# gyoge0/sub_volume_renderer

Measured on AMD Instinct MI355X. Metric: Mray-steps/sec (+ frames/sec) of the LMIP sub-volume march at 1920x1080, 3-LOD 1024^3 volume, higher is better.
Workload: dtype f32

## Files before the change

### sub_volume_renderer_amd/csrc/march_kernel.hip

```cpp
#include <stdlib.h>

#include <algorithm>
#include <type_traits>

#include "svr_internal.h"
#include "twin_address.h"
#include "slab_box.h"

namespace {

struct f3 { float x, y, z; };
struct f4 { float x, y, z, w; };

__device__ __forceinline__ f4 mat_vec(const float* m, float x, float y, float z, float w) {
    f4 r;
    r.x = ((m[0] * x + m[4] * y) + m[8]  * z) + m[12] * w;
    r.y = ((m[1] * x + m[5] * y) + m[9]  * z) + m[13] * w;
    r.z = ((m[2] * x + m[6] * y) + m[10] * z) + m[14] * w;
    r.w = ((m[3] * x + m[7] * y) + m[11] * z) + m[15] * w;
    return r;
}

__device__ __forceinline__ float dot3(f3 a, f3 b) { return (a.x * b.x + a.y * b.y) + a.z * b.z; }

// ... 467 lines not shown
                     SVR_STEP1X("quad_perm:[2,3,0,1] row_mask:0xf bank_mask:0xf")
                     SVR_STEP1X("row_half_mirror row_mask:0xf bank_mask:0xf")
                     SVR_STEP1X("row_mirror row_mask:0xf bank_mask:0xf")
                     SVR_STEP1X("row_bcast:15 row_mask:0xa bank_mask:0xf")
                     SVR_STEP1X("row_bcast:31 row_mask:0xc bank_mask:0xf")
                     "s_nop 0" : "+v"(v));
    else
        asm volatile(SVR_STEP1("quad_perm:[1,0,3,2] row_mask:0xf bank_mask:0xf")
                     SVR_STEP1("quad_perm:[2,3,0,1] row_mask:0xf bank_mask:0xf")
                     SVR_STEP1("row_half_mirror row_mask:0xf bank_mask:0xf")
                     SVR_STEP1("row_mirror row_mask:0xf bank_mask:0xf")
                     SVR_STEP1("row_bcast:15 row_mask:0xa bank_mask:0xf")
                     SVR_STEP1("row_bcast:31 row_mask:0xc bank_mask:0xf")
                     "s_nop 0" : "+v"(v));
#undef SVR_STEP1
#undef SVR_STEP1X
    return __builtin_amdgcn_readlane(v, 63);
}

struct LodK {
    uint32_t ring[3];
    float    scale[3];
    int32_t  addw[3];
    uint32_t rx4, base_bytes;
    float    ss[3];
    int32_t  slab;
    const void* rbase;
    uint32_t rbytes;
    uint32_t nparts, zsplit, part_bytes, rbytes_last;
    uint32_t twin;
};
__device__ __forceinline__ LodK load_lod(kparams_t p, int l) {
    LodK k;
#pragma unroll
    for (int a = 0; a < 3; ++a) {
        k.ring[a] = p->lod[l].ring[a]; k.scale[a] = p->lod[l].scale[a]; k.addw[a] = p->lod[l].addw[a]; k.ss[a] = p->lod[l].ss[a];
    }
    k.rx4 = p->lod[l].rx4; k.base_bytes = p->lod[l].base_bytes; k.slab = p->lod[l].slab;
    k.rbase = p->lod[l].rbase; k.rbytes = p->lod[l].rbytes;
    k.nparts = p->lod[l].nparts; k.zsplit = p->lod[l].zsplit; k.part_bytes = p->lod[l].part_bytes; k.rbytes_last = p->lod[l].rbytes_last;
    k.twin = p->lod[l].twin;
    return k;
}

struct LodEvents {
    int a, b;
    int cx, cy, cz;
};


template <int NL, int U, bool COUNT, int ESH, bool BIG, bool WAVG = false, bool SCALED = false>
__global__ __launch_bounds__(256) __attribute__((amdgpu_waves_per_eu(SCALED && !COUNT ? 5 : 1))) void march_span(const MarchParams P) {
    static_assert(!(SCALED && WAVG), "the weighted-average reducer reads the unscaled step");
    extern __shared__ __attribute__((aligned(16))) uint8_t lds_all[];
    const int nblocks = P.tiles_x * P.tiles_y;
    const int tb = P.tile_order ? (int)P.tile_order[blockIdx.x] : xcd_remap((int)blockIdx.x, nblocks);
    const int tile_x = tb % P.tiles_x, tile_y = tb / P.tiles_x;
    const int wave = __builtin_amdgcn_readfirstlane((int)(threadIdx.x >> 6)), lane = threadIdx.x & 63;
    const int lw = P.tile_log2w, wl = P.block_waves_log2;
    const int c0 = ((tile_x << wl) + (wave & wl)) << lw, r0 = ((tile_y << wl) + (wave >> 1)) << (6 - lw);
    int lc = lane & ((1 << lw) - 1), lr = lane >> lw;
    {
        const float pcx = (float)(P.frame.x0 + c0) + 0.5f * (float)(1 << lw);
        const float pcy = (float)(P.frame.y0 + (r0 / P.frame.band_h) * P.frame.band_pitch + (r0 % P.frame.band_h)) +
                          0.5f * (float)(64 >> lw);
        const float ncx = 2.0f * pcx / (float)P.frame.frame_w - 1.0f;
        const float ncy = 1.0f - 2.0f * pcy / (float)P.frame.frame_h;
        const float dx = (P.xdir[0] - ncx * P.xdir[3]) * (float)P.frame.frame_w;
        const float dy = (P.xdir[1] - ncy * P.xdir[3]) * (float)P.frame.frame_h;
        if (P.orient && fabsf(dy) > fabsf(dx)) { lr = lane & ((64 >> lw) - 1); lc = lane >> (6 - lw); }
    }
    const int c = c0 + lc;
    const int r = r0 + lr;
    const bool inside = c < P.frame.out_w && r < P.frame.out_h;
    const size_t o = (size_t)r * (size_t)P.frame.out_w + (size_t)c;
    const int x = P.frame.x0 + c;
    const int y = P.frame.y0 + (r / P.frame.band_h) * P.frame.band_pitch + (r % P.frame.band_h);

    unsigned long long t_acc[16] = { 0, 0, 0, 0, 0, 0, 0, 0, 0, 0, 0, 0, 0, 0, 0, 0 };
    unsigned long long t_last = COUNT ? __builtin_amdgcn_s_memtime() : 0ull;
    auto lap = [&](int k) {
        if (COUNT) {
            const unsigned long long t = __builtin_amdgcn_s_memtime();
            t_acc[k] += t - t_last;
            t_last = t;
        }
    };

    Ray Rs;
    Rs.nsteps = 0; Rs.start = { 0.f, 0.f, 0.f }; Rs.step = { 0.f, 0.f, 0.f };
    const bool frag = inside && (x < P.frame.frame_w && y < P.frame.frame_h) && setup_ray(P, x, y, Rs);
    const int nsteps = frag ? Rs.nsteps : 0;
    float Rsx = frag ? Rs.start.x : 0.f, Rsy = frag ? Rs.start.y : 0.f, Rsz = frag ? Rs.start.z : 0.f;
    float Rtx = frag ? Rs.step.x : 0.f, Rty = frag ? Rs.step.y : 0.f, Rtz = frag ? Rs.step.z : 0.f;

    float d0[3], d1[3];
    {
        const float lastf = (float)(nsteps - 1);
        d0[0] = (Rsx + 0.0f * Rtx) * P.size[0];  d1[0] = (Rsx + lastf * Rtx) * P.size[0];
        d0[1] = (Rsy + 0.0f * Rty) * P.size[1];  d1[1] = (Rsy + lastf * Rty) * P.size[1];
        d0[2] = (Rsz + 0.0f * Rtz) * P.size[2];  d1[2] = (Rsz + lastf * Rtz) * P.size[2];
    }
    LodEvents ev[NL];
#pragma unroll
    for (int l = 0; l < NL; ++l) {
        const LodParams& L = P.lod[l];
        int a = 0, b = nsteps, cr[3] = { 0, 0, 0 };
        if (L.shape[0] == 0 || L.shape[1] == 0 || L.shape[2] == 0) {
            ev[l].a = 0; ev[l].b = 0; ev[l].cx = 0; ev[l].cy = 0; ev[l].cz = 0;
            continue;
        }
#pragma unroll
        for (int ax = 0; ax < 3; ++ax) {
            const float st = ax == 0 ? Rsx : (ax == 1 ? Rsy : Rsz);
            const float sp = ax == 0 ? Rtx : (ax == 1 ? Rty : Rtz);
            const bool inc = sp > 0.0f;
            const int v0 = (int)(d0[ax] * L.scale[ax]), v1 = (int)(d1[ax] * L.scale[ax]);
            auto cross = [&](int T) {
                const bool p0 = inc ? v0 >= T : v0 < T;
                const bool p1 = inc ? v1 >= T : v1 < T;
                int j = p0 ? 0 : nsteps;
                const bool need = !p0 && p1;
                if (__builtin_amdgcn_ballot_w64(need) != 0) {
                    const int js = first_cross(nsteps, st, sp, P.size[ax], L.scale[ax], T, need);
                    j = need ? js : j;
                }
                return j;
            };
            const int lo = L.off[ax], hi = L.off[ax] + (int)L.shape[ax];
            const int jlo = cross(lo);
            const int jhi = cross(hi);
            int en = inc ? jlo : jhi, ex = inc ? jhi : jlo;
            if (!(sp > 0.0f) && !(sp < 0.0f)) {
                en = 0; ex = (lo <= v0 && v0 < hi) ? nsteps : 0;
            }
            a = max(a, en); b = min(b, ex);
            if (L.wrap0[ax] + L.shape[ax] > L.ring[ax])
                cr[ax] = cross((int)L.ring[ax] - L.addw[ax]);
            else
                cr[ax] = inc ? nsteps : 0;
        }
        if (a >= b || L.shape[0] == 0) { a = 0; b = 0; }
        ev[l].a = a; ev[l].b = b; ev[l].cx = cr[0]; ev[l].cy = cr[1]; ev[l].cz = cr[2];
    }

    __amdgpu_buffer_rsrc_t rsrc_all = __builtin_amdgcn_make_buffer_rsrc(
        const_cast<void*>(P.density_all), 0, (int)P.density_all_bytes, 0x00020000);

#ifdef SVR_EXPERIMENTS
    const int dbg_nowait = P.dbg_nowait, brick_pow2 = P.brick_pow2;
#else
    constexpr int dbg_nowait = 0, brick_pow2 = 0;
#endif
    bool found = false, finished = (dbg_nowait & 2) != 0;
    float local_max = 0.f, samp = 0.f;
    int hit_i = 0, since = 0;
    uint32_t steps = 0;

    typedef typename Texel<ESH>::type texel_t;
    texel_t thr_raw;
    if constexpr (ESH != 2) thr_raw = P.lmip_threshold_raw; else thr_raw = P.lmip_threshold;
    const bool mip_like = (P.skip_flags & 2) != 0;
    float den = 0.f;
    auto lmip_batch = [&](const texel_t (&sv)[U], int nb, bool live, bool tail) {
        if constexpr (WAVG) {
            const float steplen = sqrtf((Rtx * Rtx + Rty * Rty) + Rtz * Rtz);
            const float k = fresh_params(P)->weight_falloff;
#pragma unroll
            for (int u = 0; u < U; ++u) {
                const bool act = live && !finished && (!tail || (nb + u) < nsteps);
                const float tw = 1.0f - k * ((float)(nb + u) * steplen);
                const bool go = act && tw > 0.0f;
                finished = finished || (act && !go);
                if (COUNT) steps += go ? 1u : 0u;
                const float val = texel_value(sv[u]);
                const float w = tw * tw;
                const float contribution = w * fabsf(val);
                const float num1 = samp + w * val, den1 = den + w;
                samp = go ? num1 : samp;
                den = go ? den1 : den;
                const bool take = go && contribution > local_max;
                local_max = take ? contribution : local_max;
                hit_i = take ? (nb + u) : hit_i;
            }
            return;
        }
        texel_t m;
        if constexpr (ESH != 2) m = 0u; else m = -1.0f;
        const texel_t neutral = m;
#pragma unroll
        for (int u = 0; u < U; ++u) m = texel_max(m, (tail && (nb + u) >= nsteps) ? neutral : texel_abs(sv[u]));
        bool need;
        if (mip_like) need = live && (found ? texel_value(m) > local_max : m >= thr_raw);
        else need = live && (found || m >= thr_raw);
        if (__builtin_amdgcn_ballot_w64(need) != 0) {
#pragma unroll
            for (int u = 0; u < U; ++u) {
                const bool act = live && !finished && (!tail || (nb + u) < nsteps);
                const float val = texel_value(sv[u]);
                const float inten = fabsf(val);
                if (COUNT) steps += act ? 1u : 0u;
                const bool was_found = found;
                const bool first_hit = act && !was_found && inten >= P.lmip_threshold;
                const bool tracking = act && was_found;
                since += tracking ? 1 : 0;
                const bool take = first_hit || (tracking && inten > local_max);
                local_max = take ? inten : local_max;
                samp = take ? val : samp;
                hit_i = take ? (nb + u) : hit_i;
                found = found || first_hit;
                const bool brk = tracking && (since >= P.lmip_max_samples || inten < local_max * P.lmip_fall_off);
                finished = finished || brk;
            }
        } else if (COUNT) {
            steps += live ? (uint32_t)(tail ? (min(nb + U, nsteps) - nb) : U) : 0u;
        }
    };

    int code = NL, E = 0;
    uint32_t Kc = 0xFFFFFFFFu;
    uint32_t Kb = 0u;
    int zth = 0;

    int brick_mode = 0;
    bool many_lines = false;
    if (P.brick) {
        const float pf = (float)min(max(nsteps - 1, 0), 256);
        const int qx = (int)((Rsx + pf * Rtx) * P.size[0]) >> (7 - ESH);
        const int qy = (int)((Rsy + pf * Rty) * P.size[1]);
        const int qz = (int)((Rsz + pf * Rtz) * P.size[2]);
        const int key = frag ? ((qz * 4099 + qy) * 64 + (qx & 63)) : -1 - lane;
        const int k0 = __builtin_amdgcn_update_dpp(key, key, 0x00, 0xF, 0xF, false);
        const int k1 = __builtin_amdgcn_update_dpp(key, key, 0x55, 0xF, 0xF, false);
        const int k2 = __builtin_amdgcn_update_dpp(key, key, 0xAA, 0xF, 0xF, false);
        const int q = lane & 3;
        const bool fresh = frag && (q == 0 || (key != k0 && (q == 1 || (key != k1 && (q == 2 || key != k2)))));
        const int lines = __builtin_popcountll(__builtin_amdgcn_ballot_w64(fresh));
        const int quads = __builtin_popcountll(__builtin_amdgcn_ballot_w64(frag && q == 0)) + 1;
        const bool use_brick = P.brick >= 2 || lines * 16 > P.brick_lines * quads;
        brick_mode = use_brick ? 1 + P.slab_long : 0;
        many_lines = use_brick;
    }
    const int wave_lds = wave * P.brick_bytes;

    int c_general = 0, c_direct = 0, c_brick = 0, c_slabs = 0, c_runs = 0, c_zero = 0, c_skip = 0;
    int n = 0;
    lap(0);
    while (true) {
        const bool alive = !finished && n < nsteps;
        const unsigned long long alive_mask = __builtin_amdgcn_ballot_w64(alive);
        if (alive_mask == 0) break;

        if (__builtin_amdgcn_ballot_w64(alive && n >= E) != 0) {
            const kparams_t Pr = fresh_params(P);
            if (alive && n >= E) {
                code = NL; E = nsteps; Kc = 0xFFFFFFFFu;
                bool settled = false;
#pragma unroll
                for (int l = 0; l < NL; ++l) {
                    const bool in = !settled && n >= ev[l].a && n < ev[l].b;
                    if (in) {
                        const LodK L = load_lod(Pr, l);
                        code = l;
                        E = min(E, ev[l].b);
                        const bool px = (n >= ev[l].cx) == (Rtx > 0.0f);
                        const bool py = (n >= ev[l].cy) == (Rty > 0.0f);
                        const bool pz = (n >= ev[l].cz) == (Rtz > 0.0f);
                        const uint32_t kx = (uint32_t)L.addw[0] - (px ? L.ring[0] : 0u);
                        const uint32_t ky = (uint32_t)L.addw[1] - (py ? L.ring[1] : 0u);
                        const uint32_t kz = (uint32_t)L.addw[2] - (pz ? L.ring[2] : 0u);
                        Kc = (kz * L.ring[1] + ky) * L.rx4 + (kx << ESH) + L.base_bytes;
                        if (many_lines && L.twin) {
                            typedef TwinBlock<ESH> B;
                            Kb = svr_twin_lane_const<ESH>((uint32_t)(((int)kz >> B::ZB) * (int)(L.ring[1] >> B::YB) + ((int)ky >> B::YB)) * (L.ring[0] >> B::XB) +
                                                          (uint32_t)((int)kx >> B::XB));
                        }
                        if constexpr (BIG) zth = (int)L.zsplit - (int)kz;
                        if (ev[l].cx > n) E = min(E, ev[l].cx);
                        if (ev[l].cy > n) E = min(E, ev[l].cy);
                        if (ev[l].cz > n) E = min(E, ev[l].cz);
                    } else if (!settled && ev[l].a > n) {
                        E = min(E, ev[l].a);
                    }
                    settled = settled || in;
                }
            }
        }

        const int first = __builtin_amdgcn_readlane(code, (int)__builtin_ctzll(alive_mask));
        int lane_run = (code == first) ? ((E == nsteps ? E - n + U - 1 : E - n) / U) : 0;
        if (first < NL && !fresh_params(P)->lod_pow2[first < NL ? first : 0]) lane_run = alive ? 0 : lane_run;
        if (!alive) lane_run = 0x3fffffff;
        int run = wave_reduce<false>(lane_run);
        if (COUNT) ++c_runs;
        lap(1);

        if (run <= 0) {
            if (COUNT) ++c_general;
            const kparams_t Pg = fresh_params(P);
            texel_t s[U];
            const float basef = (float)n;
            if constexpr (!BIG) {
                uint32_t off[U];
#pragma unroll
                for (int u = 0; u < U; ++u) {
                    off[u] = 0xFFFFFFFFu;
                    const float iter = basef + (float)u;
                    const float dx = (Rsx + iter * Rtx) * Pg->size[0];
                    const float dy = (Rsy + iter * Rty) * Pg->size[1];
                    const float dz = (Rsz + iter * Rtz) * Pg->size[2];
                    bool done = !alive || (n + u) >= nsteps;
#pragma unroll
                    for (int l = 0; l < NL; ++l) {
                        const bool sel = !done && (n + u) >= ev[l].a && (n + u) < ev[l].b;
                        if (__builtin_amdgcn_ballot_w64(sel) != 0) {
                            const uint32_t ofs = lod_offset_wrapped<ESH>(load_lod(Pg, l), dx, dy, dz);
                            off[u] = sel ? ofs : off[u];
                        }
                        done = done || sel;
                    }
                }
#pragma unroll
                for (int u = 0; u < U; ++u) s[u] = fetch_density<ESH>(rsrc_all, off[u]);
            } else {
#pragma unroll
                for (int u = 0; u < U; ++u) {
                    const float iter = basef + (float)u;
                    const float dx = (Rsx + iter * Rtx) * Pg->size[0];
                    const float dy = (Rsy + iter * Rty) * Pg->size[1];
                    const float dz = (Rsz + iter * Rtz) * Pg->size[2];
                    bool done = !alive || (n + u) >= nsteps;
                    texel_t acc = 0;
#pragma unroll
                    for (int l = 0; l < NL; ++l) {
                        const bool sel = !done && (n + u) >= ev[l].a && (n + u) < ev[l].b;
                        if (__builtin_amdgcn_ballot_w64(sel) != 0) {
                            const LodK Lg = load_lod(Pg, l);
                            uint32_t part;
                            const uint32_t ofs = lod_offset_wrapped_split<ESH>(Lg, dx, dy, dz, part);
                            for (unsigned long long todo = __builtin_amdgcn_ballot_w64(sel); todo != 0ull;) {
                                const uint32_t p = (uint32_t)__builtin_amdgcn_readlane((int)part, (int)__builtin_ctzll(todo));
                                const bool mine = sel && part == p;
                                const texel_t t = fetch_density<ESH>(part_rsrc(Lg, p), mine ? ofs : 0xFFFFFFFFu);
                                acc = mine ? t : acc;
                                todo &= ~__builtin_amdgcn_ballot_w64(mine);
                            }
                        }
                        done = done || sel;
                    }
                    s[u] = acc;
                }
            }
            lmip_batch(s, n, alive, true);
            n += U;
            lap(2);
            continue;
        }

        if (first == NL) {
            texel_t s[U];
#pragma unroll
            for (int u = 0; u < U; ++u) s[u] = 0;
            for (; run > 0; --run) {
                if (COUNT) ++c_zero;
                const bool lv = alive && !finished && n < nsteps;
                if (__builtin_amdgcn_ballot_w64(lv && n + U > nsteps) != 0) lmip_batch(s, n, lv, true);
                else lmip_batch(s, n, lv, false);
                n += U;
                if (__builtin_amdgcn_ballot_w64(alive && !finished && n < nsteps) == 0) break;
            }
            continue;
        }

        {
            const LodK L = load_lod(fresh_params(P), first);
            const float ssx = L.ss[0], ssy = L.ss[1], ssz = L.ss[2];
            if constexpr (SCALED) { Rsx *= ssx; Rsy *= ssy; Rsz *= ssz; Rtx *= ssx; Rty *= ssy; Rtz *= ssz; }
            __amdgpu_buffer_rsrc_t rsrc = rsrc_all;
            if constexpr (BIG) rsrc = __builtin_amdgcn_make_buffer_rsrc(const_cast<void*>(L.rbase), 0, (int)L.rbytes, 0x00020000);
            const bool ring_split = BIG && L.nparts > 1u;
            const bool use_twin = many_lines && L.twin == 1u;

            int held = 0;
            do {
            run += held; held = 0;
            if (P.cells_all_bytes != 0u) {
                const kparams_t Ps = fresh_params(P);
                const int sb = Ps->lod[first].skip_batches;
                if (sb > 0 && run >= 4 * sb) {
                    const float reach = (float)(8 * sb);
                    const uint32_t cs = (uint32_t)Ps->lod[first].cshift;
                    const float vx = SCALED ? Rtx : Rtx * ssx, vy = SCALED ? Rty : Rty * ssy, vz = SCALED ? Rtz : Rtz * ssz;
                    const bool slow = fmaxf(fmaxf(fabsf(vx), fabsf(vy)), fabsf(vz)) * reach <=
                                      (float)(1u << cs) - 0.5f;
                    __amdgpu_buffer_rsrc_t crsrc = __builtin_amdgcn_make_buffer_rsrc(
                        const_cast<void*>(Ps->cells_all), 0, (int)Ps->cells_all_bytes, 0x00020000);
                    const uint32_t cbase = Ps->lod[first].cell_base;
                    const uint32_t cdx = Ps->lod[first].cdim[0], cdy = Ps->lod[first].cdim[1], cdz = Ps->lod[first].cdim[2];
                    bool vetoed = false, tracking_only = false;
                    uint32_t c0x, c0y, c0z;
                    {
                        const float i0 = fminf((float)n, (float)(nsteps - 1));
                        c0x = ((uint32_t)(int)coord_one<SCALED>(i0, Rsx, Rtx, ssx) + (uint32_t)L.addw[0]) >> cs;
                        c0y = ((uint32_t)(int)coord_one<SCALED>(i0, Rsy, Rty, ssy) + (uint32_t)L.addw[1]) >> cs;
                        c0z = ((uint32_t)(int)coord_one<SCALED>(i0, Rsz, Rtz, ssz) + (uint32_t)L.addw[2]) >> cs;
                    }
                    while (run >= 4 * sb) {
                        const bool live = alive && !finished && n < nsteps;
                        const float lastf = fminf((float)(nsteps - 1), (float)n + 4.0f * reach - (run > 4 * sb ? 0.0f : 1.0f));
                        uint32_t px[5], py[5], pz[5];
                        px[0] = c0x; py[0] = c0y; pz[0] = c0z;
#pragma unroll
                        for (int g = 1; g < 5; g += 2) {
                            const float i0 = (float)n + reach * (float)g;
                            const float2_t iter = { fminf(i0, lastf), fminf(i0 + reach, lastf) };
                            const Idx2 q = voxel_pair<SCALED>(Rsx, Rsy, Rsz, Rtx, Rty, Rtz, iter, ssx, ssy, ssz);
                            px[g] = (q.x0 + (uint32_t)L.addw[0]) >> cs; py[g] = (q.y0 + (uint32_t)L.addw[1]) >> cs; pz[g] = (q.z0 + (uint32_t)L.addw[2]) >> cs;
                            px[g + 1] = (q.x1 + (uint32_t)L.addw[0]) >> cs; py[g + 1] = (q.y1 + (uint32_t)L.addw[1]) >> cs;
                            pz[g + 1] = (q.z1 + (uint32_t)L.addw[2]) >> cs;
                        }
                        c0x = px[4]; c0y = py[4]; c0z = pz[4];
                        texel_t v[4];
#pragma unroll
                        for (int g = 0; g < 4; ++g) {
                            uint32_t bx = min(px[g], px[g + 1]), by = min(py[g], py[g + 1]), bz = min(pz[g], pz[g + 1]);
                            bx = min(bx, bx - cdx); by = min(by, by - cdy); bz = min(bz, bz - cdz);
                            v[g] = fetch_density<ESH>(crsrc, (__umul24(__umul24(bz, cdy) + by, cdx) + bx) << ESH, cbase);
                        }
                        const texel_t m = texel_max(texel_max(texel_abs(v[0]), texel_abs(v[1])), texel_max(texel_abs(v[2]), texel_abs(v[3])));
                        const bool occupied = live && !found && (!slow || m >= thr_raw);
                        const bool following = live && found && (!mip_like || !slow || texel_value(m) > local_max);
                        const unsigned long long occ_mask = __builtin_amdgcn_ballot_w64(occupied);
                        if (occ_mask != 0 || __builtin_amdgcn_ballot_w64(following) != 0) {
                            vetoed = true;
                            tracking_only = occ_mask == 0;
                            break;
                        }
                        if (COUNT) { steps += live ? (uint32_t)(min(n + 32 * sb, nsteps) - n) : 0u; c_skip += 4 * sb; }
                        n += 32 * sb;
                        run -= 4 * sb;
                        if (__builtin_amdgcn_ballot_w64(alive && !finished && n < nsteps) == 0) { run = 0; break; }
                    }
                    if (vetoed) {
                        int cap = 4 * sb;
                        if (brick_mode && L.slab > 0 && !use_twin) cap = max(cap, (L.slab << (brick_mode - 1)) / U);
                        if (tracking_only && (P.skip_flags & 1) && !mip_like) cap = min(cap, 2);
                        if (run > cap) { held = run - cap; run = cap; }
                    }
                }
                lap(10);
            }

            {
                while (brick_mode && L.slab > 0 && !use_twin && run >= (L.slab << (brick_mode - 1)) / U) {
                    const int slab = L.slab << (brick_mode - 1);
                    const bool live = alive && !finished && n < nsteps;
                    const float2_t it = { (float)n, (float)min(n + slab - 1, nsteps - 1) };
                    const float2_t ex = coord_pair<SCALED>(it, Rsx, Rtx, ssx);
                    const float2_t ey = coord_pair<SCALED>(it, Rsy, Rty, ssy);
                    const float2_t ez = coord_pair<SCALED>(it, Rsz, Rtz, ssz);
#if defined(SVR_EXPERIMENTS) && defined(SVR_EXP_NO_BOX_REDUCE)
                    const int big = 0x7fffffff;
                    int lx = live ? min((int)ex.x, (int)ex.y) : big, hx = live ? max((int)ex.x, (int)ex.y) : -big;
                    int ly = live ? min((int)ey.x, (int)ey.y) : big, hy = live ? max((int)ey.x, (int)ey.y) : -big;
                    int lz = live ? min((int)ez.x, (int)ez.y) : big, hz = live ? max((int)ez.x, (int)ez.y) : -big;
                    lx = __builtin_amdgcn_readfirstlane(lx); ly = __builtin_amdgcn_readfirstlane(ly); lz = __builtin_amdgcn_readfirstlane(lz);
                    hx = lx + 12; hy = ly + 10; hz = lz + 10;
                    const bool none_live = lx == big;
#else
                    const svr_slab_box box = svr_slab_box_reduce(svr_slab_box_pack(ex.x, ex.y, ey.x, ey.y, ez.x, ez.y, live));
                    const int lx = box.lx, ly = box.ly, lz = box.lz, hx = box.hx, hy = box.hy, hz = box.hz;
                    const bool none_live = box.none;
#endif
                    if (COUNT) ++c_slabs;
                    lap(8);
                    if (none_live) { run = 0; break; }
                    constexpr int GSH = 4 - ESH;
                    const int gx0 = lx - ((lx + L.addw[0]) & ((1 << GSH) - 1));
                    const int ngx = ((hx - gx0) >> GSH) + 1;
                    const int ny = hy - ly + 1, nz = hz - lz + 1;
                    const int gp = brick_pow2 ? (ngx <= 1 ? 1 : 1 << (32 - __builtin_clz(ngx - 1))) : (ngx | 1);
                    const int pz = brick_pow2 ? ny * gp : ((ny * gp) | 1);
                    if (ny >= 512 || pz * nz * 16 > P.brick_bytes) {
                        if (brick_mode > 1) { --brick_mode; continue; }
                        brick_mode = 0; break;
                    }
                    const float rgp = __builtin_amdgcn_rcpf((float)gp);
                    const int ly_lane = (int)(((float)lane + 0.5f) * rgp);
                    const int rows_per = __builtin_amdgcn_readlane(ly_lane, 63) + ((gp & (gp - 1)) == 0 && gp <= 64 ? 1 : 0);
                    const int g_lane = lane - __mul24(ly_lane, gp);
                    uint32_t wx = (uint32_t)(gx0 + (g_lane << GSH) + L.addw[0]);
                    wx = min(wx, wx - L.ring[0]);
                    wx <<= ESH;
                    const uint32_t plane_bytes = (uint32_t)(pz << 4);
                    const uint32_t zpitch = L.ring[1] * L.rx4;
                    lap(9);
#if defined(SVR_EXPERIMENTS) && defined(SVR_EXP_NO_BRICK_LOADS)
                    if (false)
#endif
                    for (int yc = 0; yc < ny; yc += rows_per) {
                        const int yy = yc + ly_lane;
                        uint32_t wy = (uint32_t)(ly + yy + L.addw[1]);
                        wy = min(wy, wy - L.ring[1]);
                        const uint32_t lane_src = mad24(wy, L.rx4, L.base_bytes + wx);
                        const uint32_t lds_chunk = (uint32_t)wave_lds + (uint32_t)((yc * gp) << 4);
                        if (yy < ny && g_lane < ngx && ly_lane < rows_per) {
                            for (int zz = 0; zz < nz; ++zz) {
                                uint32_t wz = (uint32_t)(lz + zz + L.addw[2]);
                                wz = min(wz, wz - L.ring[2]);
                                if (BIG && ring_split) {
                                    uint32_t p = 0u;
                                    while (p + 1u < L.nparts && wz >= (p + 1u) * L.zsplit) ++p;
                                    __builtin_amdgcn_raw_ptr_buffer_load_lds(
                                        part_rsrc(L, p), (__attribute__((address_space(3))) void*)(lds_all + lds_chunk + zz * plane_bytes),
                                        16, (int)(lane_src + (wz - p * L.zsplit) * zpitch), 0, 0, 0);
                                } else
                                __builtin_amdgcn_raw_ptr_buffer_load_lds(
                                    rsrc, (__attribute__((address_space(3))) void*)(lds_all + lds_chunk + zz * plane_bytes),
                                    16, (int)(lane_src + wz * zpitch), 0, 0, 0);
                            }
                        }
                    }
                    const uint32_t lds_base = (uint32_t)reinterpret_cast<uintptr_t>((__attribute__((address_space(3))) uint8_t*)lds_all);
                    const uint32_t bk = lds_base + (uint32_t)wave_lds - (uint32_t)(((lz * pz + ly * gp) << 4) + (gx0 << ESH));
                    lap(3);
                    if (!(dbg_nowait & 1)) asm volatile("s_waitcnt vmcnt(0)" ::: "memory");
                    lap(4);
                    const uint32_t kyz = (uint32_t)(gp << 4) | ((uint32_t)(pz << 4) << 16);
                    const bool slab_tail = __builtin_amdgcn_ballot_w64(live && n + slab > nsteps) != 0;
                    for (int k = 0; k < slab / U; ++k) {
                        texel_t s[U];
                        float2_t iter = { (float)n, (float)n + 1.0f };
#pragma unroll
                        for (int u = 0; u < U; u += 2) {
                            const Idx2p v = voxel_pair_packed<SCALED>(Rsx, Rsy, Rsz, Rtx, Rty, Rtz, iter, ssx, ssy, ssz);
                            iter += 2.0f;
                            const uint32_t a0 = dot2_u16(v.yz0, kyz, shl_add_c<ESH>(v.x0, bk));
                            const uint32_t a1 = dot2_u16(v.yz1, kyz, shl_add_c<ESH>(v.x1, bk));
                            s[u] = lds_texel<ESH>(a0);
                            s[u + 1] = lds_texel<ESH>(a1);
                        }
                        if constexpr (ESH != 2 && U == 8)
                            asm("" : "+v"(s[0]), "+v"(s[1]), "+v"(s[2]), "+v"(s[3]), "+v"(s[4]), "+v"(s[5]), "+v"(s[6]), "+v"(s[7]));
                        {
                            const bool lv = alive && !finished && n < nsteps;
                            if (slab_tail && __builtin_amdgcn_ballot_w64(lv && n + U > nsteps) != 0) lmip_batch(s, n, lv, true);
                            else lmip_batch(s, n, lv, false);
                        }
                        n += U;
                        if (COUNT) ++c_brick;
                    }
                    run -= slab / U;
                    lap(5);
                    asm volatile("" ::: "memory");
                }
            }

            __amdgpu_buffer_rsrc_t rsrc_twin = rsrc;
            const void* twin_base = nullptr;
            uint32_t twin_w = 0u;
            auto direct_batches = [&](auto from_twin) {
            constexpr int TWF = decltype(from_twin)::value;
            constexpr bool TW = TWF != 0;
            for (; run > 0; --run) {
                const bool live = alive && !finished && n < nsteps;
                if (__builtin_amdgcn_ballot_w64(live) == 0) break;
                if (COUNT) { ++c_direct; if (TW) t_acc[15] += 1ull; }
                texel_t s[U];
                uint32_t off[U];
                float2_t iter = { (float)n, (float)n + 1.0f };
                if constexpr (TWF == 2) {
#pragma unroll
                    for (int u = 0; u < U; u += 2) {
                        const Idx2p v = voxel_pair_packed<SCALED>(Rsx, Rsy, Rsz, Rtx, Rty, Rtz, iter, ssx, ssy, ssz);
                        iter += 2.0f;
                        off[u] = svr_twin_offset<ESH>(v.x0, v.yz0, twin_w, Kb);
                        off[u + 1] = svr_twin_offset<ESH>(v.x1, v.yz1, twin_w, Kb);
                    }
                } else if constexpr (TWF == 1) {
                    const TwinConsts tc = twin_consts<ESH>(L.ring[0], L.ring[1]);
                    const uint32_t KbS = Kb << TwinBlock<ESH>::SZ;
#pragma unroll
                    for (int u = 0; u < U; u += 2) {
                        const Idx2p v = voxel_pair_packed<SCALED>(Rsx, Rsy, Rsz, Rtx, Rty, Rtz, iter, ssx, ssy, ssz);
                        iter += 2.0f;
                        off[u] = twin_offset_packed<ESH>(v.x0, v.yz0, tc, KbS);
                        off[u + 1] = twin_offset_packed<ESH>(v.x1, v.yz1, tc, KbS);
                    }
                } else {
#pragma unroll
                for (int u = 0; u < U; u += 2) {
                    const Idx2 v = voxel_pair<SCALED>(Rsx, Rsy, Rsz, Rtx, Rty, Rtz, iter, ssx, ssy, ssz);
                    iter += 2.0f;
                    off[u] = mad24(mad24(v.z0, L.ring[1], v.y0), L.rx4, shl_add_c<ESH>(v.x0, Kc));
                    off[u + 1] = mad24(mad24(v.z1, L.ring[1], v.y1), L.rx4, shl_add_c<ESH>(v.x1, Kc));
                }
                }
#pragma unroll
                for (int u = 0; u < U; ++u) s[u] = undefined_value<texel_t>();
                if (BIG && ring_split) {
                    auto part_of = [&](int icz) {
                        uint32_t q = 0u;
                        for (uint32_t k = 1; k < L.nparts; ++k) q += icz >= zth + (int)((k - 1u) * L.zsplit) ? 1u : 0u;
                        return q;
                    };
                    const float2_t ends = { (float)n, (float)min(n + U - 1, nsteps - 1) };
                    const float2_t ez2 = coord_pair<SCALED>(ends, Rsz, Rtz, ssz);
                    const uint32_t pa = part_of((int)ez2.x), pb = part_of((int)ez2.y);
                    const uint32_t p0 = (uint32_t)__builtin_amdgcn_readlane((int)pa, (int)__builtin_ctzll(__builtin_amdgcn_ballot_w64(live)));
                    if (__builtin_amdgcn_ballot_w64(live && (pa != p0 || pb != p0)) == 0) {
                        const __amdgpu_buffer_rsrc_t rp = part_rsrc(L, p0, TW ? twin_base : L.rbase);
                        const uint32_t sub = p0 * L.part_bytes;
#pragma unroll
                        for (int u = 0; u < U; ++u) s[u] = fetch_density<ESH>(rp, live ? off[u] - sub : 0xFFFFFFFFu);
                    } else {
                    float2_t it2 = { (float)n, (float)n + 1.0f };
#pragma unroll
                    for (int u = 0; u < U; u += 2) {
                        const float2_t cz = coord_pair<SCALED>(it2, Rsz, Rtz, ssz);
                        it2 += 2.0f;
#pragma unroll
                        for (int h = 0; h < 2; ++h) {
                            const int icz = h ? (int)cz.y : (int)cz.x;
                            uint32_t part = 0u;
                            for (uint32_t k = 1; k < L.nparts; ++k) part += icz >= zth + (int)((k - 1u) * L.zsplit) ? 1u : 0u;
                            const uint32_t rel = off[u + h] - part * L.part_bytes;
                            texel_t a = 0;
                            for (unsigned long long todo = __builtin_amdgcn_ballot_w64(live); todo != 0ull;) {
                                const uint32_t p = (uint32_t)__builtin_amdgcn_readlane((int)part, (int)__builtin_ctzll(todo));
                                const bool mine = live && part == p;
                                const texel_t t = fetch_density<ESH>(part_rsrc(L, p, TW ? twin_base : L.rbase), mine ? rel : 0xFFFFFFFFu);
                                a = mine ? t : a;
                                todo &= ~__builtin_amdgcn_ballot_w64(mine);
                            }
                            s[u + h] = a;
                        }
                    }
                    }
                } else
                if (live) {
#pragma unroll
                    for (int u = 0; u < U; ++u) s[u] = fetch_density<ESH>(TW ? rsrc_twin : rsrc, off[u]);
                }
                if (__builtin_amdgcn_ballot_w64(live && n + U > nsteps) != 0) lmip_batch(s, n, live, true);
                else lmip_batch(s, n, live, false);
                n += U;
            }
            };
            if (use_twin || (many_lines && L.twin == 2u && (brick_mode == 0 || L.slab <= 0))) {
                const kparams_t Pt = fresh_params(P);
                twin_base = Pt->lod[first].twin_rbase;
                rsrc_twin = __builtin_amdgcn_make_buffer_rsrc(const_cast<void*>(twin_base), 0, (int)Pt->lod[first].twin_rbytes, 0x00020000);
                if constexpr (ESH != 2) twin_w = Pt->lod[first].twin_w;
                if (ESH != 2 && twin_w != 0u) direct_batches(std::integral_constant<int, 2>{});
                else direct_batches(std::integral_constant<int, 1>{});
            } else {
                direct_batches(std::integral_constant<int, 0>{});
            }
            } while (held > 0 && __builtin_amdgcn_ballot_w64(alive && !finished && n < nsteps) != 0);
            if constexpr (SCALED) {
                const kparams_t Pu = fresh_params(P);
                const float ux = Pu->lod[first].rss[0], uy = Pu->lod[first].rss[1], uz = Pu->lod[first].rss[2];
                Rsx *= ux; Rsy *= uy; Rsz *= uz; Rtx *= ux; Rty *= uy; Rtz *= uz;
            }
            lap(6);
        }
    }

    if (COUNT && P.dbg && lane == 0) {
        atomicAdd(P.dbg + 0, (uint32_t)c_general); atomicAdd(P.dbg + 1, (uint32_t)c_direct);
        atomicAdd(P.dbg + 2, (uint32_t)c_brick);   atomicAdd(P.dbg + 3, (uint32_t)c_slabs);
        atomicAdd(P.dbg + 4, (uint32_t)c_runs);    atomicAdd(P.dbg + 5, (uint32_t)c_zero);
        atomicAdd(P.dbg + 6, 1u);                  atomicAdd(P.dbg + 7, (uint32_t)c_skip);
    }
    Hit h;
    h.found = found; h.sample = samp; h.steps = steps;
    if constexpr (WAVG) { h.found = local_max > 0.0f; h.sample = h.found ? samp / den : 0.0f; }
    const float hit_f = (float)hit_i;
    h.offset = { hit_f * Rtx, hit_f * Rty, hit_f * Rtz };
    h.coord = { Rsx + h.offset.x, Rsy + h.offset.y, Rsz + h.offset.z };
    if (inside) {
#if defined(__HIP_DEVICE_COMPILE__)
        const MarchParams* Pk = (const MarchParams*)__builtin_amdgcn_kernarg_segment_ptr();
        asm volatile("" : "+s"(Pk));
#else
        const MarchParams* Pk = &P;
#endif
        shade_and_store<NL>(*Pk, o, frag, h);
        if (COUNT && Pk->steps) Pk->steps[o] = h.steps;
    }
    if (COUNT && P.dbg) {
        lap(7);
        if (lane == 0) {
            unsigned long long* t_out = reinterpret_cast<unsigned long long*>(P.dbg + 8);
#pragma unroll
            for (int k = 0; k < 16; ++k) atomicAdd(t_out + k, t_acc[k]);
        }
    }
}

template <int NL>
hipError_t launch_nl(const MarchParams& p, int kind, hipStream_t stream) {
    const int nblocks = p.tiles_x * p.tiles_y;
    if (nblocks <= 0) return hipSuccess;
    const bool simple = kind == 1 || !p.span_ok;
    const bool wavg = p.render_mode == SVR_MODE_WEIGHTED_AVERAGE;
    if (wavg && (simple || p.per_lod_rsrc)) {
        if (p.steps) hipLaunchKernelGGL((march_wavg<NL, true>), dim3(nblocks), dim3(256), 0, stream, p);
        else         hipLaunchKernelGGL((march_wavg<NL, false>), dim3(nblocks), dim3(256), 0, stream, p);
    } else if (simple) {
        if (p.steps) hipLaunchKernelGGL((march_simple<NL, true>), dim3(nblocks), dim3(256), 0, stream, p);
        else         hipLaunchKernelGGL((march_simple<NL, false>), dim3(nblocks), dim3(256), 0, stream, p);
    } else {
        const int threads = 64 << (2 * p.block_waves_log2);
        const size_t lds = (size_t)p.brick_bytes * (threads / 64);
#define SVR_LAUNCH_SPAN_SC(ESH_, SC_)                                                                                              \
    do {                                                                                                                           \
        if (p.per_lod_rsrc) {                                                                                                      \
            if (p.steps) hipLaunchKernelGGL((march_span<NL, 8, true, ESH_, true>), dim3(nblocks), dim3(threads), lds, stream, p);   \
            else         hipLaunchKernelGGL((march_span<NL, 8, false, ESH_, true>), dim3(nblocks), dim3(threads), lds, stream, p);  \
        } else {                                                                                                                   \
            if (p.steps) hipLaunchKernelGGL((march_span<NL, 8, true, ESH_, false, false, SC_>), dim3(nblocks), dim3(threads), lds, stream, p);  \
            else         hipLaunchKernelGGL((march_span<NL, 8, false, ESH_, false, false, SC_>), dim3(nblocks), dim3(threads), lds, stream, p); \
        }                                                                                                                          \
    } while (0)
#define SVR_LAUNCH_SPAN(ESH_)                                                                                              \
    do {                                                                                                                   \
        if (p.ss_pow2 && !p.per_lod_rsrc) SVR_LAUNCH_SPAN_SC(ESH_, true);                                                  \
        else           SVR_LAUNCH_SPAN_SC(ESH_, false);                                                                    \
    } while (0)
#define SVR_LAUNCH_WAVG(ESH_)                                                                                              \
    do {                                                                                                                   \
        if (p.steps) hipLaunchKernelGGL((march_span<NL, 8, true, ESH_, false, true>), dim3(nblocks), dim3(threads), lds, stream, p);   \
        else         hipLaunchKernelGGL((march_span<NL, 8, false, ESH_, false, true>), dim3(nblocks), dim3(threads), lds, stream, p);  \
    } while (0)
        if (wavg) {
            if (p.density_esh == 0) SVR_LAUNCH_WAVG(0);
            else if (p.density_esh == 1) SVR_LAUNCH_WAVG(1);
            else SVR_LAUNCH_WAVG(2);
        }
        else if (p.density_esh == 0) SVR_LAUNCH_SPAN(0);
        else if (p.density_esh == 1) SVR_LAUNCH_SPAN(1);
        else SVR_LAUNCH_SPAN(2);
#undef SVR_LAUNCH_WAVG
#undef SVR_LAUNCH_SPAN
#undef SVR_LAUNCH_SPAN_SC
    }
    return hipGetLastError();
}

}

#ifndef SVR_NL
#error "compile with -DSVR_NL=<number of LODs>"
#endif
#define SVR_CAT2(a, b) a##b
#define SVR_CAT(a, b) SVR_CAT2(a, b)
hipError_t SVR_CAT(svr_launch_march_nl, SVR_NL)(const MarchParams& p, int kind, hipStream_t stream) {
    return launch_nl<SVR_NL>(p, kind, stream);
}
```

Before: 2.025 million.

## Track per-lane found/finished state as wave-wide scalar masks in march loop

Replaces the per-lane bool found/finished flags with 64-bit wave masks held in scalar registers, built with ballot and read back with inverse_ballot. Liveness and tail checks become mask arithmetic, and for integer texel paths the step counter and iteration coordinates are carried as wave-uniform offsets from a base. The aim is to move control state and branch conditions off vector registers and VALU compares onto the scalar unit, and to drop redundant ballots per batch. It adds considerable complexity to the LMIP state machine, with a risk of subtle divergence in termination semantics.

```diff
diff --git a/sub_volume_renderer_amd/csrc/march_kernel.hip b/sub_volume_renderer_amd/csrc/march_kernel.hip
--- a/sub_volume_renderer_amd/csrc/march_kernel.hip
+++ b/sub_volume_renderer_amd/csrc/march_kernel.hip
@@ -643,7 +643,15 @@
 #else
     constexpr int dbg_nowait = 0, brick_pow2 = 0;
 #endif
-    bool found = false, finished = (dbg_nowait & 2) != 0;
+    typedef unsigned long long mask_t;
+    mask_t found_m = 0ull, fin_m = (dbg_nowait & 2) != 0 ? ~0ull : 0ull;
+    auto live_at = [&](int i) -> mask_t { return __builtin_amdgcn_ballot_w64(i < nsteps) & ~fin_m; };
+    constexpr bool kCarryIter = !WAVG && ESH != 2;
+    constexpr bool kLaneBools = WAVG || ESH == 2;
+    constexpr bool kScalarCount = !kLaneBools;
+    auto live_in = [&](int nb, int rem, int k8) -> mask_t {
+        return (kScalarCount ? __builtin_amdgcn_ballot_w64(k8 < rem) : __builtin_amdgcn_ballot_w64(nb < nsteps)) & ~fin_m;
+    };
     float local_max = 0.f, samp = 0.f;
     int hit_i = 0, since = 0;
     uint32_t steps = 0;
@@ -653,58 +661,122 @@
     if constexpr (ESH != 2) thr_raw = P.lmip_threshold_raw; else thr_raw = P.lmip_threshold;
     const bool mip_like = (P.skip_flags & 2) != 0;
     float den = 0.f;
-    auto lmip_batch = [&](const texel_t (&sv)[U], int nb, bool live, bool tail) {
-        if constexpr (WAVG) {
-            const float steplen = sqrtf((Rtx * Rtx + Rty * Rty) + Rtz * Rtz);
-            const float k = fresh_params(P)->weight_falloff;
-#pragma unroll
-            for (int u = 0; u < U; ++u) {
-                const bool act = live && !finished && (!tail || (nb + u) < nsteps);
-                const float tw = 1.0f - k * ((float)(nb + u) * steplen);
-                const bool go = act && tw > 0.0f;
-                finished = finished || (act && !go);
-                if (COUNT) steps += go ? 1u : 0u;
-                const float val = texel_value(sv[u]);
-                const float w = tw * tw;
-                const float contribution = w * fabsf(val);
-                const float num1 = samp + w * val, den1 = den + w;
-                samp = go ? num1 : samp;
-                den = go ? den1 : den;
-                const bool take = go && contribution > local_max;
-                local_max = take ? contribution : local_max;
-                hit_i = take ? (nb + u) : hit_i;
-            }
+    auto lmip_batch = [&](const texel_t (&sv)[U], int nb, mask_t live_m) {
+        if constexpr (kLaneBools) {
+            auto body = [&](auto tail_c) {
+                constexpr bool tail = decltype(tail_c)::value;
+                const bool live = __builtin_amdgcn_inverse_ballot_w64(live_m);
+                bool found = __builtin_amdgcn_inverse_ballot_w64(found_m), finished = __builtin_amdgcn_inverse_ballot_w64(fin_m);
+                if constexpr (WAVG) {
+                    const float steplen = sqrtf((Rtx * Rtx + Rty * Rty) + Rtz * Rtz);
+                    const float k = fresh_params(P)->weight_falloff;
+#pragma unroll
+                    for (int u = 0; u < U; ++u) {
+                        const bool act = live && !finished && (!tail || (nb + u) < nsteps);
+                        const float tw = 1.0f - k * ((float)(nb + u) * steplen);
+                        const bool go = act && tw > 0.0f;
+                        finished = finished || (act && !go);
+                        if (COUNT) steps += go ? 1u : 0u;
+                        const float val = texel_value(sv[u]);
+                        const float w = tw * tw;
+                        const float contribution = w * fabsf(val);
+                        const float num1 = samp + w * val, den1 = den + w;
+                        samp = go ? num1 : samp;
+                        den = go ? den1 : den;
+                        const bool take = go && contribution > local_max;
+                        local_max = take ? contribution : local_max;
+                        hit_i = take ? (nb + u) : hit_i;
+                    }
+                    fin_m = __builtin_amdgcn_ballot_w64(finished);
+                    return;
+                }
+                texel_t m;
+                if constexpr (ESH != 2) m = 0u; else m = -1.0f;
+                const texel_t neutral = m;
+#pragma unroll
+                for (int u = 0; u < U; ++u) m = texel_max(m, (tail && (nb + u) >= nsteps) ? neutral : texel_abs(sv[u]));
+                bool need;
+                if (mip_like) need = live && (found ? texel_value(m) > local_max : m >= thr_raw);
+                else need = live && (found || m >= thr_raw);
+                if (__builtin_amdgcn_ballot_w64(need) != 0) {
+#pragma unroll
+                    for (int u = 0; u < U; ++u) {
+                        const bool act = live && !finished && (!tail || (nb + u) < nsteps);
+                        const float val = texel_value(sv[u]);
+                        const float inten = fabsf(val);
+                        if (COUNT) steps += act ? 1u : 0u;
+                        const bool was_found = found;
+                        const bool first_hit = act && !was_found && inten >= P.lmip_threshold;
+                        const bool tracking = act && was_found;
+                        since += tracking ? 1 : 0;
+                        const bool take = first_hit || (tracking && inten > local_max);
+                        local_max = take ? inten : local_max;
+                        samp = take ? val : samp;
+                        hit_i = take ? (nb + u) : hit_i;
+                        found = found || first_hit;
+                        const bool brk = tracking && (since >= P.lmip_max_samples || inten < local_max * P.lmip_fall_off);
+                        finished = finished || brk;
+                    }
+                    found_m = __builtin_amdgcn_ballot_w64(found);
+                    fin_m = __builtin_amdgcn_ballot_w64(finished);
+                } else if (COUNT) {
+                    steps += live ? (uint32_t)(tail ? (min(nb + U, nsteps) - nb) : U) : 0u;
+                }
+            };
+            if ((live_m & __builtin_amdgcn_ballot_w64(nb + U > nsteps)) != 0) body(std::true_type{});
+            else body(std::false_type{});
             return;
         }
         texel_t m;
         if constexpr (ESH != 2) m = 0u; else m = -1.0f;
         const texel_t neutral = m;
 #pragma unroll
-        for (int u = 0; u < U; ++u) m = texel_max(m, (tail && (nb + u) >= nsteps) ? neutral : texel_abs(sv[u]));
-        bool need;
-        if (mip_like) need = live && (found ? texel_value(m) > local_max : m >= thr_raw);
-        else need = live && (found || m >= thr_raw);
-        if (__builtin_amdgcn_ballot_w64(need) != 0) {
-#pragma unroll
-            for (int u = 0; u < U; ++u) {
-                const bool act = live && !finished && (!tail || (nb + u) < nsteps);
-                const float val = texel_value(sv[u]);
-                const float inten = fabsf(val);
-                if (COUNT) steps += act ? 1u : 0u;
-                const bool was_found = found;
-                const bool first_hit = act && !was_found && inten >= P.lmip_threshold;
-                const bool tracking = act && was_found;
-                since += tracking ? 1 : 0;
-                const bool take = first_hit || (tracking && inten > local_max);
-                local_max = take ? inten : local_max;
-                samp = take ? val : samp;
-                hit_i = take ? (nb + u) : hit_i;
-                found = found || first_hit;
-                const bool brk = tracking && (since >= P.lmip_max_samples || inten < local_max * P.lmip_fall_off);
-                finished = finished || brk;
-            }
+        for (int u = 0; u < U; ++u) m = texel_max(m, texel_abs(sv[u]));
+        if (((__builtin_amdgcn_ballot_w64(m >= thr_raw) | found_m) & live_m) != 0) {
+            auto machine = [&](auto tail_c) {
+                constexpr bool tail = decltype(tail_c)::value;
+                mask_t in_m[U];
+                if (tail) {
+                    m = neutral;
+#pragma unroll
+                    for (int u = 0; u < U; ++u) {
+                        in_m[u] = __builtin_amdgcn_ballot_w64((nb + u) < nsteps);
+                        m = texel_max(m, __builtin_amdgcn_inverse_ballot_w64(in_m[u]) ? texel_abs(sv[u]) : neutral);
+                    }
+                }
+                mask_t need_m = found_m;
+                if (tail || mip_like) {
+                    if (mip_like) need_m &= __builtin_amdgcn_ballot_w64(texel_value(m) > local_max);
+                    need_m |= __builtin_amdgcn_ballot_w64(m >= thr_raw) & ~found_m;
+                    if ((need_m & live_m) == 0) return false;
+                }
+#pragma unroll
+                for (int u = 0; u < U; ++u) {
+                    mask_t act_m = live_m & ~fin_m;
+                    if (tail) act_m &= in_m[u];
+                    const float val = texel_value(sv[u]);
+                    const float inten = fabsf(val);
+                    if (COUNT) steps += __builtin_amdgcn_inverse_ballot_w64(act_m) ? 1u : 0u;
+                    const mask_t first_m = act_m & ~found_m & __builtin_amdgcn_ballot_w64(inten >= P.lmip_threshold);
+                    const mask_t track_m = act_m & found_m;
+                    since += __builtin_amdgcn_inverse_ballot_w64(track_m) ? 1 : 0;
+                    const bool take = __builtin_amdgcn_inverse_ballot_w64(
+                        first_m | (track_m & __builtin_amdgcn_ballot_w64(inten > local_max)));
+                    local_max = take ? inten : local_max;
+                    samp = take ? val : samp;
+                    hit_i = take ? (nb + u) : hit_i;
+                    found_m |= first_m;
+                    fin_m |= track_m & (__builtin_amdgcn_ballot_w64(since >= P.lmip_max_samples) |
+                                        __builtin_amdgcn_ballot_w64(inten < local_max * P.lmip_fall_off));
+                }
+                return true;
+            };
+            bool ran;
+            if ((live_m & __builtin_amdgcn_ballot_w64(nb + U > nsteps)) != 0) ran = machine(std::true_type{});
+            else ran = machine(std::false_type{});
+            if (COUNT && !ran) steps += __builtin_amdgcn_inverse_ballot_w64(live_m) ? (uint32_t)(min(nb + U, nsteps) - nb) : 0u;
         } else if (COUNT) {
-            steps += live ? (uint32_t)(tail ? (min(nb + U, nsteps) - nb) : U) : 0u;
+            steps += __builtin_amdgcn_inverse_ballot_w64(live_m) ? (uint32_t)(min(nb + U, nsteps) - nb) : 0u;
         }
     };
 
@@ -738,13 +810,14 @@
     int n = 0;
     lap(0);
     while (true) {
-        const bool alive = !finished && n < nsteps;
-        const unsigned long long alive_mask = __builtin_amdgcn_ballot_w64(alive);
+        const mask_t alive_mask = live_at(n);
         if (alive_mask == 0) break;
-
-        if (__builtin_amdgcn_ballot_w64(alive && n >= E) != 0) {
+        const bool alive = __builtin_amdgcn_inverse_ballot_w64(alive_mask);
+
+        const mask_t refresh_m = alive_mask & __builtin_amdgcn_ballot_w64(n >= E);
+        if (refresh_m != 0) {
             const kparams_t Pr = fresh_params(P);
-            if (alive && n >= E) {
+            if (__builtin_amdgcn_inverse_ballot_w64(refresh_m)) {
                 code = NL; E = nsteps; Kc = 0xFFFFFFFFu;
                 bool settled = false;
 #pragma unroll
@@ -842,7 +915,7 @@
                     s[u] = acc;
                 }
             }
-            lmip_batch(s, n, alive, true);
+            lmip_batch(s, n, alive_mask);
             n += U;
             lap(2);
             continue;
@@ -852,13 +925,10 @@
             texel_t s[U];
 #pragma unroll
             for (int u = 0; u < U; ++u) s[u] = 0;
-            for (; run > 0; --run) {
+            for (mask_t lv_m = alive_mask; run > 0 && lv_m != 0; --run, lv_m = live_at(n)) {
                 if (COUNT) ++c_zero;
-                const bool lv = alive && !finished && n < nsteps;
-                if (__builtin_amdgcn_ballot_w64(lv && n + U > nsteps) != 0) lmip_batch(s, n, lv, true);
-                else lmip_batch(s, n, lv, false);
+                lmip_batch(s, n, lv_m);
                 n += U;
-                if (__builtin_amdgcn_ballot_w64(alive && !finished && n < nsteps) == 0) break;
             }
             continue;
         }
@@ -882,8 +952,8 @@
                     const float reach = (float)(8 * sb);
                     const uint32_t cs = (uint32_t)Ps->lod[first].cshift;
                     const float vx = SCALED ? Rtx : Rtx * ssx, vy = SCALED ? Rty : Rty * ssy, vz = SCALED ? Rtz : Rtz * ssz;
-                    const bool slow = fmaxf(fmaxf(fabsf(vx), fabsf(vy)), fabsf(vz)) * reach <=
-                                      (float)(1u << cs) - 0.5f;
+                    const mask_t slow_m = __builtin_amdgcn_ballot_w64(fmaxf(fmaxf(fabsf(vx), fabsf(vy)), fabsf(vz)) * reach <=
+                                                                      (float)(1u << cs) - 0.5f);
                     __amdgpu_buffer_rsrc_t crsrc = __builtin_amdgcn_make_buffer_rsrc(
                         const_cast<void*>(Ps->cells_all), 0, (int)Ps->cells_all_bytes, 0x00020000);
                     const uint32_t cbase = Ps->lod[first].cell_base;
@@ -897,7 +967,7 @@
                         c0z = ((uint32_t)(int)coord_one<SCALED>(i0, Rsz, Rtz, ssz) + (uint32_t)L.addw[2]) >> cs;
                     }
                     while (run >= 4 * sb) {
-                        const bool live = alive && !finished && n < nsteps;
+                        const mask_t live_m = live_at(n);
                         const float lastf = fminf((float)(nsteps - 1), (float)n + 4.0f * reach - (run > 4 * sb ? 0.0f : 1.0f));
                         uint32_t px[5], py[5], pz[5];
                         px[0] = c0x; py[0] = c0y; pz[0] = c0z;
@@ -919,18 +989,18 @@
                             v[g] = fetch_density<ESH>(crsrc, (__umul24(__umul24(bz, cdy) + by, cdx) + bx) << ESH, cbase);
                         }
                         const texel_t m = texel_max(texel_max(texel_abs(v[0]), texel_abs(v[1])), texel_max(texel_abs(v[2]), texel_abs(v[3])));
-                        const bool occupied = live && !found && (!slow || m >= thr_raw);
-                        const bool following = live && found && (!mip_like || !slow || texel_value(m) > local_max);
-                        const unsigned long long occ_mask = __builtin_amdgcn_ballot_w64(occupied);
-                        if (occ_mask != 0 || __builtin_amdgcn_ballot_w64(following) != 0) {
+                        const mask_t occ_mask = live_m & ~found_m & (~slow_m | __builtin_amdgcn_ballot_w64(m >= thr_raw));
+                        mask_t fol_mask = live_m & found_m;
+                        if (mip_like && fol_mask != 0) fol_mask &= ~slow_m | __builtin_amdgcn_ballot_w64(texel_value(m) > local_max);
+                        if ((occ_mask | fol_mask) != 0) {
                             vetoed = true;
                             tracking_only = occ_mask == 0;
                             break;
                         }
-                        if (COUNT) { steps += live ? (uint32_t)(min(n + 32 * sb, nsteps) - n) : 0u; c_skip += 4 * sb; }
+                        if (COUNT) { steps += __builtin_amdgcn_inverse_ballot_w64(live_m) ? (uint32_t)(min(n + 32 * sb, nsteps) - n) : 0u; c_skip += 4 * sb; }
                         n += 32 * sb;
                         run -= 4 * sb;
-                        if (__builtin_amdgcn_ballot_w64(alive && !finished && n < nsteps) == 0) { run = 0; break; }
+                        if (live_at(n) == 0) { run = 0; break; }
                     }
                     if (vetoed) {
                         int cap = 4 * sb;
@@ -945,7 +1015,7 @@
             {
                 while (brick_mode && L.slab > 0 && !use_twin && run >= (L.slab << (brick_mode - 1)) / U) {
                     const int slab = L.slab << (brick_mode - 1);
-                    const bool live = alive && !finished && n < nsteps;
+                    const bool live = __builtin_amdgcn_inverse_ballot_w64(live_at(n));
                     const float2_t it = { (float)n, (float)min(n + slab - 1, nsteps - 1) };
                     const float2_t ex = coord_pair<SCALED>(it, Rsx, Rtx, ssx);
                     const float2_t ey = coord_pair<SCALED>(it, Rsy, Rty, ssy);
@@ -1018,10 +1088,12 @@
                     if (!(dbg_nowait & 1)) asm volatile("s_waitcnt vmcnt(0)" ::: "memory");
                     lap(4);
                     const uint32_t kyz = (uint32_t)(gp << 4) | ((uint32_t)(pz << 4) << 16);
-                    const bool slab_tail = __builtin_amdgcn_ballot_w64(live && n + slab > nsteps) != 0;
-                    for (int k = 0; k < slab / U; ++k) {
+                    float2_t iter = { (float)n, (float)n + 1.0f };
+                    const int n0 = n, rem = kScalarCount ? nsteps - n0 : 0;
+                    for (int k8 = 0; k8 < slab; k8 += U) {
                         texel_t s[U];
-                        float2_t iter = { (float)n, (float)n + 1.0f };
+                        const int nb = kScalarCount ? n0 + k8 : n;
+                        if constexpr (!kCarryIter) iter = float2_t{ (float)nb, (float)nb + 1.0f };
 #pragma unroll
                         for (int u = 0; u < U; u += 2) {
                             const Idx2p v = voxel_pair_packed<SCALED>(Rsx, Rsy, Rsz, Rtx, Rty, Rtz, iter, ssx, ssy, ssz);
@@ -1033,14 +1105,11 @@
                         }
                         if constexpr (ESH != 2 && U == 8)
                             asm("" : "+v"(s[0]), "+v"(s[1]), "+v"(s[2]), "+v"(s[3]), "+v"(s[4]), "+v"(s[5]), "+v"(s[6]), "+v"(s[7]));
-                        {
-                            const bool lv = alive && !finished && n < nsteps;
-                            if (slab_tail && __builtin_amdgcn_ballot_w64(lv && n + U > nsteps) != 0) lmip_batch(s, n, lv, true);
-                            else lmip_batch(s, n, lv, false);
-                        }
-                        n += U;
+                        lmip_batch(s, nb, live_in(nb, rem, k8));
+                        if constexpr (!kScalarCount) n += U;
                         if (COUNT) ++c_brick;
                     }
+                    if constexpr (kScalarCount) n = n0 + slab;
                     run -= slab / U;
                     lap(5);
                     asm volatile("" ::: "memory");
@@ -1053,13 +1122,18 @@
             auto direct_batches = [&](auto from_twin) {
             constexpr int TWF = decltype(from_twin)::value;
             constexpr bool TW = TWF != 0;
-            for (; run > 0; --run) {
-                const bool live = alive && !finished && n < nsteps;
-                if (__builtin_amdgcn_ballot_w64(live) == 0) break;
+            float2_t iter = { (float)n, (float)n + 1.0f };
+            const int n0 = n, rem = kScalarCount ? nsteps - n0 : 0;
+            int k8 = 0;
+            for (; run > 0; --run, k8 += U) {
+                const int nb = kScalarCount ? n0 + k8 : n;
+                const mask_t live_m = live_in(nb, rem, k8);
+                if (live_m == 0) break;
+                const bool live = __builtin_amdgcn_inverse_ballot_w64(live_m);
                 if (COUNT) { ++c_direct; if (TW) t_acc[15] += 1ull; }
                 texel_t s[U];
                 uint32_t off[U];
-                float2_t iter = { (float)n, (float)n + 1.0f };
+                if constexpr (!kCarryIter) iter = float2_t{ (float)nb, (float)nb + 1.0f };
                 if constexpr (TWF == 2) {
 #pragma unroll
                     for (int u = 0; u < U; u += 2) {
@@ -1095,17 +1169,17 @@
                         for (uint32_t k = 1; k < L.nparts; ++k) q += icz >= zth + (int)((k - 1u) * L.zsplit) ? 1u : 0u;
                         return q;
                     };
-                    const float2_t ends = { (float)n, (float)min(n + U - 1, nsteps - 1) };
+                    const float2_t ends = { (float)nb, (float)min(nb + U - 1, nsteps - 1) };
                     const float2_t ez2 = coord_pair<SCALED>(ends, Rsz, Rtz, ssz);
                     const uint32_t pa = part_of((int)ez2.x), pb = part_of((int)ez2.y);
-                    const uint32_t p0 = (uint32_t)__builtin_amdgcn_readlane((int)pa, (int)__builtin_ctzll(__builtin_amdgcn_ballot_w64(live)));
+                    const uint32_t p0 = (uint32_t)__builtin_amdgcn_readlane((int)pa, (int)__builtin_ctzll(live_m));
                     if (__builtin_amdgcn_ballot_w64(live && (pa != p0 || pb != p0)) == 0) {
                         const __amdgpu_buffer_rsrc_t rp = part_rsrc(L, p0, TW ? twin_base : L.rbase);
                         const uint32_t sub = p0 * L.part_bytes;
 #pragma unroll
                         for (int u = 0; u < U; ++u) s[u] = fetch_density<ESH>(rp, live ? off[u] - sub : 0xFFFFFFFFu);
                     } else {
-                    float2_t it2 = { (float)n, (float)n + 1.0f };
+                    float2_t it2 = { (float)nb, (float)nb + 1.0f };
 #pragma unroll
                     for (int u = 0; u < U; u += 2) {
                         const float2_t cz = coord_pair<SCALED>(it2, Rsz, Rtz, ssz);
@@ -1117,7 +1191,7 @@
                             for (uint32_t k = 1; k < L.nparts; ++k) part += icz >= zth + (int)((k - 1u) * L.zsplit) ? 1u : 0u;
                             const uint32_t rel = off[u + h] - part * L.part_bytes;
                             texel_t a = 0;
-                            for (unsigned long long todo = __builtin_amdgcn_ballot_w64(live); todo != 0ull;) {
+                            for (unsigned long long todo = live_m; todo != 0ull;) {
                                 const uint32_t p = (uint32_t)__builtin_amdgcn_readlane((int)part, (int)__builtin_ctzll(todo));
                                 const bool mine = live && part == p;
                                 const texel_t t = fetch_density<ESH>(part_rsrc(L, p, TW ? twin_base : L.rbase), mine ? rel : 0xFFFFFFFFu);
@@ -1133,10 +1207,10 @@
 #pragma unroll
                     for (int u = 0; u < U; ++u) s[u] = fetch_density<ESH>(TW ? rsrc_twin : rsrc, off[u]);
                 }
-                if (__builtin_amdgcn_ballot_w64(live && n + U > nsteps) != 0) lmip_batch(s, n, live, true);
-                else lmip_batch(s, n, live, false);
-                n += U;
+                lmip_batch(s, nb, live_m);
+                if constexpr (!kScalarCount) n += U;
             }
+            if constexpr (kScalarCount) n = n0 + k8;
             };
             if (use_twin || (many_lines && L.twin == 2u && (brick_mode == 0 || L.slab <= 0))) {
                 const kparams_t Pt = fresh_params(P);
@@ -1148,7 +1222,7 @@
             } else {
                 direct_batches(std::integral_constant<int, 0>{});
             }
-            } while (held > 0 && __builtin_amdgcn_ballot_w64(alive && !finished && n < nsteps) != 0);
+            } while (held > 0 && live_at(n) != 0);
             if constexpr (SCALED) {
                 const kparams_t Pu = fresh_params(P);
                 const float ux = Pu->lod[first].rss[0], uy = Pu->lod[first].rss[1], uz = Pu->lod[first].rss[2];
@@ -1165,7 +1239,7 @@
         atomicAdd(P.dbg + 6, 1u);                  atomicAdd(P.dbg + 7, (uint32_t)c_skip);
     }
     Hit h;
-    h.found = found; h.sample = samp; h.steps = steps;
+    h.found = __builtin_amdgcn_inverse_ballot_w64(found_m); h.sample = samp; h.steps = steps;
     if constexpr (WAVG) { h.found = local_max > 0.0f; h.sample = h.found ? samp / den : 0.0f; }
     const float hit_f = (float)hit_i;
     h.offset = { hit_f * Rtx, hit_f * Rty, hit_f * Rtz };
```

Result: faster. 2.266 million, median of 6 (+11.9%).
